# qcraftai/gedepth

Measured on AMD Instinct MI355X. Metric: training img/s (whole node), KITTI-shaped 352x1120 synthetic batches, higher is better.
Workload: dtype bf16; 1 GPU; depthformer_swint_v: DepthFormer-SwinT + GEDepth-Vanilla, 352x1120, 8 img/GPU, full train step; global_batch=8, parallelism=dp1, allreduce_dtype=fp32, layout=nhwc, window_attention=bf16 mfma, params=53516992, hip_graph=off

## Files before the change

### gedepth_amd/csrc/conv1x1_wgrad.hip

```cpp
#include "common.h"
#include <algorithm>

#define C1_ROWS 64
#define C1_MAX_CB 16
#define C1_MAX_IB 3
#define C1_TPW 6
#define C1_DY_PIECES 8
#define C1_X_PIECES 2

__global__ void __launch_bounds__(512, 1) conv1x1_wgrad_k(const bf16_t* __restrict__ x, const bf16_t* __restrict__ dy, float* __restrict__ dw, long M,
                                                          int Ci, int Co, int ci_chunk, int ksplit) {
  __shared__ __attribute__((aligned(16))) bf16_t dy_t[C1_MAX_CB * C1_ROWS * 32];
  __shared__ __attribute__((aligned(16))) bf16_t x_t[C1_MAX_IB * C1_ROWS * 32];
  const int tid = threadIdx.x, lane = tid & 63;
  const int wv = __builtin_amdgcn_readfirstlane(tid >> 6);
  const int ci0 = blockIdx.x * ci_chunk, co0 = blockIdx.y * (C1_MAX_CB * 32);
  const int nib = std::min(ci_chunk, Ci - ci0) >> 5, ncb = std::min(C1_MAX_CB * 32, Co - co0) >> 5;
  const int T = ncb * nib;

  int dy_row[C1_DY_PIECES], dy_col[C1_DY_PIECES], dy_lds[C1_DY_PIECES], x_row[C1_X_PIECES], x_col[C1_X_PIECES], x_lds[C1_X_PIECES];
#pragma unroll
  for (int i = 0; i < C1_DY_PIECES; ++i) {
    const int p = tid + i * 512, ppr = 4 * ncb;
    const int row = p / ppr, part = p - row * ppr;
    dy_row[i] = row < C1_ROWS ? row : -1;
    dy_col[i] = co0 + part * 8;
    dy_lds[i] = ((part >> 2) * C1_ROWS + row) * 32 + (part & 3) * 8;
  }
#pragma unroll
  for (int i = 0; i < C1_X_PIECES; ++i) {
    const int p = tid + i * 512, ppr = 4 * nib;
    const int row = p / ppr, part = p - row * ppr;
    x_row[i] = row < C1_ROWS ? row : -1;
    x_col[i] = ci0 + part * 8;
    x_lds[i] = ((part >> 2) * C1_ROWS + row) * 32 + (part & 3) * 8;
  }
  const int tr_off = ((lane >> 5) * 8 + ((lane & 15) >> 2)) * 32 + ((lane >> 4) & 1) * 16 + (lane & 3) * 4;
  int a_off[C1_TPW], b_off[C1_TPW];
#pragma unroll
  for (int j = 0; j < C1_TPW; ++j) {
    const int t = wv + 8 * j, cb = t / nib, ib = t - cb * nib;
    a_off[j] = cb * C1_ROWS * 32 + tr_off;
    b_off[j] = ib * C1_ROWS * 32 + tr_off;
  }
  ge_f32x16 acc[C1_TPW];
#pragma unroll
  for (int j = 0; j < C1_TPW; ++j) acc[j] = 0.f;

  uint4 pd[C1_DY_PIECES], px[C1_X_PIECES];
  const uint4 zero4 = make_uint4(0, 0, 0, 0);
  const long nstage = (M + C1_ROWS - 1) / C1_ROWS;
#define C1_PREFETCH(S)                                                                                      \
  {                                                                                                         \
    const long r0_ = (long)(S) * C1_ROWS;                                                                   \
    _Pragma("unroll") for (int i = 0; i < C1_DY_PIECES; ++i) {                                             \
      pd[i] = zero4;                                                                                        \
      if (dy_row[i] >= 0 && r0_ + dy_row[i] < M) pd[i] = *(const uint4*)(dy + (r0_ + dy_row[i]) * Co + dy_col[i]);   \
    }                                                                                                       \
    _Pragma("unroll") for (int i = 0; i < C1_X_PIECES; ++i) {                                              \
      px[i] = zero4;                                                                                        \
      if (x_row[i] >= 0 && r0_ + x_row[i] < M) px[i] = *(const uint4*)(x + (r0_ + x_row[i]) * Ci + x_col[i]);        \
    }                                                                                                       \
  }
#define C1_PARK()                                                                                           \
  _Pragma("unroll") for (int i = 0; i < C1_DY_PIECES; ++i) { if (dy_row[i] >= 0) *(uint4*)(dy_t + dy_lds[i]) = pd[i]; }   \
  _Pragma("unroll") for (int i = 0; i < C1_X_PIECES; ++i) { if (x_row[i] >= 0) *(uint4*)(x_t + x_lds[i]) = px[i]; }
#define C1_RD(P) __builtin_shufflevector(__builtin_amdgcn_ds_read_tr16_b64_v4bf16(GE_LDS(ge_bf16x4, (P))), \
                                         __builtin_amdgcn_ds_read_tr16_b64_v4bf16(GE_LDS(ge_bf16x4, (P) + 4 * 32)), 0, 1, 2, 3, 4, 5, 6, 7)
  long s = blockIdx.z;
  if (s < nstage) {
    C1_PREFETCH(s)
    C1_PARK()
  }
  __syncthreads();
  for (; s < nstage; s += ksplit) {
    const bool more = s + ksplit < nstage;
    if (more) { C1_PREFETCH(s + ksplit) }
#pragma unroll
    for (int ks = 0; ks < C1_ROWS / 16; ++ks) {
#pragma unroll
      for (int j = 0; j < C1_TPW; ++j) {
        if (wv + 8 * j < T) {
          const ge_bf16x8 A = C1_RD(dy_t + a_off[j] + ks * 16 * 32);
          const ge_bf16x8 B = C1_RD(x_t + b_off[j] + ks * 16 * 32);
          acc[j] = __builtin_amdgcn_mfma_f32_32x32x16_bf16(A, B, acc[j], 0, 0, 0);
        }
      }
    }
    __syncthreads();
    if (more) { C1_PARK() }
    __syncthreads();
  }
#undef C1_PREFETCH
#undef C1_PARK
#undef C1_RD
#pragma unroll
  for (int j = 0; j < C1_TPW; ++j) {
    const int t = wv + 8 * j;
    if (t < T) {
      const int cb = t / nib, ib = t - cb * nib;
      const int ci = ci0 + ib * 32 + (lane & 31);
#pragma unroll
      for (int r = 0; r < 16; ++r) {
        const int co = co0 + cb * 32 + (r & 3) + 8 * (r >> 2) + 4 * (lane >> 5);
        atomicAdd(dw + (long)co * Ci + ci, acc[j][r]);
      }
    }
  }
}

extern "C" int ge_conv1x1_nhwc_wgrad(const void* x, const void* dy, float* dw, long M, int Cin, int Cout, int dtype, void* stream) {
  if (!x || !dy || !dw || M < 0 || Cin <= 0 || Cout <= 0) return GE_ERR_BAD_ARG;
  if (dtype != GE_BF16 || Cout % 32 || (Cin % 64 && Cin % 96) || (((uintptr_t)x | (uintptr_t)dy) & 15)) return GE_ERR_UNSUPPORTED;
  if (M == 0) return GE_OK;
  const int ci_chunk = (Cin % 96 == 0) ? 96 : 64;
  const int n_ci = Cin / ci_chunk, n_co = (Cout + C1_MAX_CB * 32 - 1) / (C1_MAX_CB * 32);
  if (n_ci > 65535 || n_co > 65535) return GE_ERR_UNSUPPORTED;
  const int cus = ge_cu_count();
  if (!cus) return GE_ERR_BAD_ARG;
  const long nstage = (M + C1_ROWS - 1) / C1_ROWS;
  long ksplit = cus / ((long)n_ci * n_co);
  ksplit = std::max(1L, std::min(ksplit, std::min(nstage, 65535L)));
  const dim3 grid((unsigned)n_ci, (unsigned)n_co, (unsigned)ksplit);
  conv1x1_wgrad_k<<<grid, 512, 0, ge_stream(stream)>>>((const bf16_t*)x, (const bf16_t*)dy, dw, M, Cin, Cout, ci_chunk, (int)ksplit);
  GE_LAUNCH_CHECK();
  return GE_OK;
}
```

### gedepth_amd/hip.py

```python
import ctypes
import os
import re

import torch

_HERE = os.path.dirname(os.path.abspath(__file__))
LIB_PATH = os.environ.get('GE_LIB') or os.path.join(_HERE, 'csrc', 'libgedepth_hip.so')
HEADERS = {'SIGNATURES': 'gedepth_hip.h', 'EVAL_SIGNATURES': 'gedepth_eval.h', 'DDAD_SIGNATURES': 'gedepth_ddad.h',
           'CLOUD_SIGNATURES': 'gedepth_cloud.h', 'GROUND_SIGNATURES': 'gedepth_ground.h'}
EXTRA_HEADERS = {'BATCH_SIGNATURES': 'gedepth_batch.h'}
SCENE_HEADERS = {'SCENE_SIGNATURES': 'gedepth_scene.h'}
STRATA_HEADERS = {'STRATA_SIGNATURES': 'gedepth_strata.h'}
GE_F32, GE_BF16 = 0, 1
GE_COLORIZE_VMIN_DATA, GE_COLORIZE_VMAX_DATA, GE_COLORIZE_EQUAL = 1, 2, 4

_SCALARS = {'int': ctypes.c_int, 'long': ctypes.c_long, 'float': ctypes.c_float, 'double': ctypes.c_double, 'size_t': ctypes.c_size_t,
            'uint64_t': ctypes.c_ulonglong, 'unsigned long long': ctypes.c_ulonglong}
_DECL = re.compile(r'\b(int|size_t)\s+(ge_\w+)\s*\(([^()]*)\)\s*;')


def parse_header(text):
    text = re.sub(r'/\*.*?\*/|//[^\n]*', ' ', text, flags=re.S)
    sigs = {}
    for res, name, params in _DECL.findall(text):
        args = []
        for p in ([] if params.strip() == 'void' else params.split(',')):
            if '*' in p:
                args.append(ctypes.c_void_p)
                continue
            ctype = ' '.join(w for w in p.split()[:-1] if w != 'const')
            if ctype not in _SCALARS:
                raise TypeError(f'{name}: parameter "{" ".join(p.split())}" has a type the ctypes binding does not map')
            args.append(_SCALARS[ctype])
        sigs[name] = (_SCALARS[res], args)
    stray = set(re.findall(r'\b(ge_\w+)\s*\(', text)) - set(sigs)
    if stray:
        raise TypeError(f'cannot parse the declaration of {", ".join(sorted(stray))}')
    return sigs


for _table, _header in {**HEADERS, **EXTRA_HEADERS, **SCENE_HEADERS, **STRATA_HEADERS}.items():
    with open(os.path.join(os.path.dirname(_HERE), 'include', _header)) as _fh:
        globals()[_table] = parse_header(_fh.read())

_lib = None


class HipLibraryError(RuntimeError):
    pass


def lib():
    global _lib
    if _lib is None:
        if not os.path.isfile(LIB_PATH):
            raise HipLibraryError(
                f'{LIB_PATH} is missing: the gfx950 HIP kernels are not built. '
                f'Run gedepth_amd/csrc/build.sh (hipcc --offload-arch=gfx950). There is no CPU/eager fallback.')
        handle = ctypes.CDLL(LIB_PATH)
        for table in (*HEADERS, *EXTRA_HEADERS, *SCENE_HEADERS, *STRATA_HEADERS):
            for name, (res, args) in globals()[table].items():
                fn = getattr(handle, name)
                fn.restype, fn.argtypes = res, args
        _lib = handle
        if os.environ.get('GE_MSDA_MODE'):
            handle.ge_msda_mode(int(os.environ['GE_MSDA_MODE']))
    return _lib


def is_built():
    return os.path.isfile(LIB_PATH)


def check(code, what):
    if code != 0:
        raise RuntimeError(f'{what} failed with code {code} '
                           f'({"bad argument" if code == 10001 else "unsupported" if code == 10002 else "hipError_t"})')


def call(name, *args):
    code = getattr(_lib or lib(), name)(*args)
    if code:
        check(code, name)


def dtype_code(t):
    if t.dtype == torch.float32:
        return GE_F32
    if t.dtype == torch.bfloat16:
        return GE_BF16
    raise TypeError(f'gedepth_amd kernels take float32 or bfloat16 tensors, got {t.dtype}')


def ptr(t, dtype=None, name='tensor'):
    if t is None:
        return None
    if not t.is_cuda:
        raise RuntimeError(f'{name}: gedepth_amd ops run on MI355X only; got a {t.device} tensor '
                           '(the CPU oracle lives in oracle/ and is test infrastructure)')
    if not t.is_contiguous():
        raise RuntimeError(f'{name} must be contiguous')
    if dtype is not None and t.dtype != dtype:
        raise TypeError(f'{name} must be {dtype}, got {t.dtype}')
    return t.data_ptr()


def stream():
    return torch.cuda.current_stream().cuda_stream
```

### gedepth_amd/mmrt/bricks.py

```python
import math
import warnings

import torch
import torch.nn as nn
import torch.nn.functional as F

from .registry import Registry, build_from_cfg

MODELS = Registry('model')
ATTENTION = Registry('attention')
POSITIONAL_ENCODING = Registry('position encoding')
DROPOUT_LAYERS = Registry('drop out layers')


def constant_init(module, val, bias=0):
    if hasattr(module, 'weight') and module.weight is not None:
        nn.init.constant_(module.weight, val)
    if hasattr(module, 'bias') and module.bias is not None:
        nn.init.constant_(module.bias, bias)


def xavier_init(module, gain=1, bias=0, distribution='normal'):
    assert distribution in ['uniform', 'normal']
    if hasattr(module, 'weight') and module.weight is not None:
        if distribution == 'uniform':
            nn.init.xavier_uniform_(module.weight, gain=gain)
        else:
            nn.init.xavier_normal_(module.weight, gain=gain)
    if hasattr(module, 'bias') and module.bias is not None:
        nn.init.constant_(module.bias, bias)


def kaiming_init(module, a=0, mode='fan_out', nonlinearity='relu', bias=0, distribution='normal'):
    assert distribution in ['uniform', 'normal']
    if hasattr(module, 'weight') and module.weight is not None:
        if distribution == 'uniform':
            nn.init.kaiming_uniform_(module.weight, a=a, mode=mode, nonlinearity=nonlinearity)
        else:
            nn.init.kaiming_normal_(module.weight, a=a, mode=mode, nonlinearity=nonlinearity)
    if hasattr(module, 'bias') and module.bias is not None:
        nn.init.constant_(module.bias, bias)


def trunc_normal_init(module, mean=0., std=1., a=-2., b=2., bias=0.):
    if isinstance(module, torch.Tensor):
        nn.init.trunc_normal_(module, mean, std, a, b)
        return
    if hasattr(module, 'weight') and module.weight is not None:
        nn.init.trunc_normal_(module.weight, mean, std, a, b)
    if hasattr(module, 'bias') and module.bias is not None:
        nn.init.constant_(module.bias, bias)


class BaseModule(nn.Module):

    def __init__(self, init_cfg=None):
        super().__init__()
        self._is_init = False
        self.init_cfg = init_cfg

    @property
    def is_init(self):
        return self._is_init

    def init_weights(self):
        if self._is_init:
            warnings.warn(f'init_weights of {self.__class__.__name__} has been called more than once.')
            return
        for m in self.children():
            if hasattr(m, 'init_weights'):
                m.init_weights()
        self._is_init = True


class Sequential(BaseModule, nn.Sequential):

    def __init__(self, *args, init_cfg=None):
        BaseModule.__init__(self, init_cfg)
        nn.Sequential.__init__(self, *args)


class ModuleList(BaseModule, nn.ModuleList):

    def __init__(self, modules=None, init_cfg=None):
        BaseModule.__init__(self, init_cfg)
        nn.ModuleList.__init__(self, modules)


def _split_k(tokens):
    if tokens < 8192:
        return 0
    for s in range(64, 3, -1):
        if tokens % s == 0 and tokens // s >= 1024:
            return s
    return 0


def _linear_fwd(xc, wc, weight, bias, dt):
    from .. import kernels
    from .optim import lowp
    K = xc.shape[-1]
    M = xc.numel() // K
    if (dt == torch.bfloat16 and xc.is_cuda and xc.is_contiguous() and wc.is_contiguous() and kernels.gemm_own(M, K, wc.shape[0])
            and (bias is None or (bias.dtype == torch.float32 and bias.is_contiguous() and bias.data_ptr() % 16 == 0))
            and xc.data_ptr() % 16 == 0 and wc.data_ptr() % 16 == 0):
        return kernels.gemm_nt(xc.reshape(M, K), wc, None if bias is None else bias.detach()).view(*xc.shape[:-1], wc.shape[0])
    return F.linear(xc, wc, None if bias is None else lowp(bias, dt))


def _linear_dx(dy2, wc):
    from .. import kernels
    M, N = dy2.shape
    K = wc.shape[1]
    if dy2.dtype == torch.bfloat16 and dy2.is_contiguous() and dy2.data_ptr() % 16 == 0 and kernels.gemm_own(M, N, K):
        return kernels.gemm_nt(dy2, wc.t().contiguous(), None)
    return dy2 @ wc


def _sum_partials(part, weight, w_dtype):
    if weight is not None and w_dtype == torch.float32:
        from .optim import grad_target
        out = grad_target(weight)
        if out is not None and out.shape == part.shape[1:]:
            return torch.sum(part, 0, dtype=torch.float32, out=out)
    return part.sum(0, dtype=torch.float32).to(w_dtype)


def _plain_dw(dy2, x2, weight, w_dtype):
    if dy2.dtype == torch.bfloat16 and x2.dtype == torch.bfloat16 and w_dtype == torch.float32:
        from .. import kernels
        if 'mm_fp32_out' not in kernels.DISABLED:
            from .optim import grad_target
            out = grad_target(weight) if weight is not None else None
            if out is not None and tuple(out.shape) == (dy2.shape[1], x2.shape[1]):
                return torch.mm(dy2.t(), x2, out_dtype=torch.float32, out=out)
            return torch.mm(dy2.t(), x2, out_dtype=torch.float32)
    return _finished_grad(dy2.t() @ x2, weight, w_dtype)


def _finished_grad(dw, weight, w_dtype):
    from .optim import grad_into_arena
    return grad_into_arena(weight, dw, w_dtype) if weight is not None else dw.to(w_dtype)


class _LinearTokens(torch.autograd.Function):

    @staticmethod
    def forward(ctx, x, weight, bias, splits):
        dt = torch.get_autocast_dtype('cuda') if torch.is_autocast_enabled() else x.dtype
        with torch.autocast('cuda', enabled=False):
            from .optim import lowp
            xc, wc = x.to(dt), lowp(weight, dt)
            y = _linear_fwd(xc, wc, weight, bias, dt)
        ctx.save_for_backward(xc, wc)
        ctx.meta = (splits, x.dtype, weight.dtype, None if bias is None else bias.dtype)
        ctx.weight_ref = weight if isinstance(weight, nn.Parameter) else None
        return y

    @staticmethod
    def backward(ctx, dy):
        xc, wc = ctx.saved_tensors
        splits, x_dtype, w_dtype, b_dtype = ctx.meta
        K = xc.numel() // xc.shape[-1]
        with torch.autocast('cuda', enabled=False):
            dy2 = dy.to(wc.dtype).reshape(K, -1)
            x2 = xc.reshape(K, -1)
            dx = dw = db = None
            if not dy2.is_contiguous():
                dy2 = dy2.contiguous()
            if ctx.needs_input_grad[0]:
                dx = _linear_dx(dy2, wc).reshape(xc.shape).to(x_dtype)
            if ctx.needs_input_grad[1]:
                if splits:
                    M, N = dy2.shape[1], x2.shape[1]
                    part = torch.bmm(dy2.view(splits, K // splits, M).transpose(1, 2), x2.view(splits, K // splits, N))
                    dw = _sum_partials(part, ctx.weight_ref, w_dtype)
                else:
                    dw = _plain_dw(dy2, x2, ctx.weight_ref, w_dtype)
            if b_dtype is not None and ctx.needs_input_grad[2]:
                if dy2.shape[1] % (4 if dy2.dtype == torch.float32 else 8) == 0:
                    from .. import kernels
                    db = kernels.colsum(dy2 if dy2.is_contiguous() else dy2.contiguous()).to(b_dtype)
                else:
                    db = dy2.sum(0, dtype=torch.float32).to(b_dtype)
        return dx, dw, db, None


class _LinearBiasGelu(torch.autograd.Function):

    @staticmethod
    def forward(ctx, x, weight, bias, splits):
        from .. import kernels
        dt = torch.get_autocast_dtype('cuda') if torch.is_autocast_enabled() else x.dtype
        with torch.autocast('cuda', enabled=False):
            from .optim import lowp
            xc, wc = x.to(dt), lowp(weight, dt)
            y0 = _linear_fwd(xc, wc, weight, bias, dt)
            g = kernels.bias_gelu_fwd(y0, None)
        ctx.save_for_backward(xc, wc, y0)
        ctx.meta = (splits, x.dtype, weight.dtype, bias.dtype)
        ctx.weight_ref = weight if isinstance(weight, nn.Parameter) else None
        return g

    @staticmethod
    def backward(ctx, dg):
        from .. import kernels
        xc, wc, y0 = ctx.saved_tensors
        splits, x_dtype, w_dtype, b_dtype = ctx.meta
        K = xc.numel() // xc.shape[-1]
        with torch.autocast('cuda', enabled=False):
            dg2 = dg.to(wc.dtype).reshape(K, -1)
            if not dg2.is_contiguous():
                dg2 = dg2.contiguous()
            dy2, db = kernels.bias_gelu_bwd(dg2, y0.reshape(K, -1), None)
            x2 = xc.reshape(K, -1)
            dx = dw = None
            if ctx.needs_input_grad[0]:
                dx = _linear_dx(dy2, wc).reshape(xc.shape).to(x_dtype)
            if ctx.needs_input_grad[1]:
                if splits:
                    M, N = dy2.shape[1], x2.shape[1]
                    part = torch.bmm(dy2.view(splits, K // splits, M).transpose(1, 2), x2.view(splits, K // splits, N))
                    dw = _sum_partials(part, ctx.weight_ref, w_dtype)
                else:
                    dw = _plain_dw(dy2, x2, ctx.weight_ref, w_dtype)
        return dx, dw, (db.to(b_dtype) if ctx.needs_input_grad[2] else None), None


def linear_bias_gelu(x, weight, bias):
    C = weight.shape[0]
    ok = (x.is_cuda and torch.is_grad_enabled() and weight.requires_grad and bias is not None and x.dim() >= 2 and x.numel() > 0
          and x.dtype in (torch.float32, torch.bfloat16) and C % 8 == 0)
    if ok:
        from .. import kernels
        ok = 'bias_gelu' not in kernels.DISABLED
    if not ok:
        return F.gelu(linear_tokens(x, weight, bias))
    return _LinearBiasGelu.apply(x, weight, bias, _split_k(x.numel() // x.shape[-1]))


def linear_tokens(x, weight, bias=None):
    if not (x.is_cuda and torch.is_grad_enabled() and weight.requires_grad) or x.dtype not in (torch.float32, torch.bfloat16) or x.dim() < 2 or x.numel() == 0:
        return F.linear(x, weight, bias)
    return _LinearTokens.apply(x, weight, bias, _split_k(x.numel() // x.shape[-1]))


class Linear(nn.Linear):

    def forward(self, x):
        return linear_tokens(x, self.weight, self.bias)


class LayerNorm(nn.LayerNorm):
    autocast_out = True

    def _hip_ok(self, x):
        C = x.shape[-1]
        return (x.is_cuda and self.elementwise_affine and len(self.normalized_shape) == 1 and C % 4 == 0 and C <= 3072
                and x.dtype in (torch.float32, torch.bfloat16))

    def _out_dtype(self, x):
        if torch.is_autocast_enabled():
            return torch.get_autocast_dtype('cuda') if self.autocast_out else torch.float32
        return x.dtype

    def forward_with_skip(self, x):
        if self._hip_ok(x) and torch.is_grad_enabled() and x.requires_grad:
            from .. import kernels
            if 'ln_res' not in kernels.DISABLED:
                return kernels.layer_norm_res(x, self.weight, self.bias, self.eps, self._out_dtype(x))
        return self(x), x

    def forward(self, x):
        C = x.shape[-1]
        if self._hip_ok(x):
            from .. import kernels
            return kernels.layer_norm(x, self.weight, self.bias, self.eps, self._out_dtype(x))
        if x.is_cuda:
            from .. import kernels
            kernels.note_fallback('LayerNorm', f'C={C} dtype={x.dtype}')
        return super().forward(x)


_NORM = {
    'BN': ('bn', nn.BatchNorm2d), 'BN1d': ('bn', nn.BatchNorm1d), 'BN2d': ('bn', nn.BatchNorm2d),
    'SyncBN': ('bn', nn.SyncBatchNorm), 'GN': ('gn', nn.GroupNorm), 'LN': ('ln', LayerNorm),
    'IN': ('in', nn.InstanceNorm2d),
}
_ACT = {
    'ReLU': nn.ReLU, 'LeakyReLU': nn.LeakyReLU, 'PReLU': nn.PReLU, 'ReLU6': nn.ReLU6, 'ELU': nn.ELU,
    'Sigmoid': nn.Sigmoid, 'Tanh': nn.Tanh, 'GELU': nn.GELU,
}
_CONV = {'Conv1d': nn.Conv1d, 'Conv2d': nn.Conv2d, 'Conv3d': nn.Conv3d, 'Conv': nn.Conv2d}


def build_norm_layer(cfg, num_features, postfix=''):
    if not isinstance(cfg, dict) or 'type' not in cfg:
        raise KeyError('the cfg dict must contain the key "type"')
    cfg_ = dict(cfg)
    layer_type = cfg_.pop('type')
    if layer_type not in _NORM:
        raise KeyError(f'Unrecognized norm type {layer_type}')
    abbr, norm_layer = _NORM[layer_type]
    name = abbr + str(postfix)
    requires_grad = cfg_.pop('requires_grad', True)
    cfg_.setdefault('eps', 1e-5)
    if layer_type == 'GN':
        assert 'num_groups' in cfg_
        layer = norm_layer(num_channels=num_features, **cfg_)
    else:
        layer = norm_layer(num_features, **cfg_)
    for p in layer.parameters():
        p.requires_grad = requires_grad
    return name, layer


def build_activation_layer(cfg):
    cfg_ = dict(cfg)
    t = cfg_.pop('type')
    if t not in _ACT:
        raise KeyError(f'Unrecognized activation type {t}')
    return _ACT[t](**cfg_)


def build_conv_layer(cfg, *args, **kwargs):
    cfg_ = dict(type='Conv2d') if cfg is None else dict(cfg)
    t = cfg_.pop('type')
    if t not in _CONV:
        raise KeyError(f'Unrecognized conv type {t}')
    return _CONV[t](*args, **kwargs, **cfg_)


class ConvModule(nn.Module):

    def __init__(self, in_channels, out_channels, kernel_size, stride=1, padding=0, dilation=1, groups=1,
                 bias='auto', conv_cfg=None, norm_cfg=None, act_cfg=dict(type='ReLU'), inplace=True,
                 order=('conv', 'norm', 'act')):
        super().__init__()
        assert order == ('conv', 'norm', 'act'), 'only the conv-norm-act order is on the GEDepth path'
        self.conv_cfg, self.norm_cfg, self.act_cfg = conv_cfg, norm_cfg, act_cfg
        self.inplace = inplace
        self.with_norm = norm_cfg is not None
        self.with_activation = act_cfg is not None
        if bias == 'auto':
            bias = not self.with_norm
        self.with_bias = bias
        self.conv = build_conv_layer(conv_cfg, in_channels, out_channels, kernel_size, stride=stride,
                                     padding=padding, dilation=dilation, groups=groups, bias=bias)
        self.in_channels, self.out_channels = in_channels, out_channels
        if self.with_norm:
            self.norm_name, norm = build_norm_layer(norm_cfg, out_channels)
            self.add_module(self.norm_name, norm)
        else:
            self.norm_name = None
        if self.with_activation:
            act_cfg_ = dict(act_cfg)
            if act_cfg_['type'] not in ['Tanh', 'PReLU', 'Sigmoid', 'GELU']:
                act_cfg_.setdefault('inplace', inplace)
            self.activate = build_activation_layer(act_cfg_)
        self.init_weights()

    @property
    def norm(self):
        return getattr(self, self.norm_name) if self.norm_name else None

    def init_weights(self):
        if self.with_activation and self.act_cfg['type'] == 'LeakyReLU':
            nonlinearity, a = 'leaky_relu', self.act_cfg.get('negative_slope', 0.01)
        else:
            nonlinearity, a = 'relu', 0
        kaiming_init(self.conv, a=a, nonlinearity=nonlinearity)
        if self.with_norm:
            constant_init(self.norm, 1, bias=0)
# ... 202 lines not shown
```

### gedepth_amd/mmrt/optim.py

```python
import math

import torch

from .. import hip


class GradArena:

    def __init__(self, params, align=64, adopt=None):
        self.params = [p for p in params if p.requires_grad]
        assert self.params, 'no trainable parameters'
        dev, dt = self.params[0].device, torch.float32
        assert all(p.dtype == dt and p.device == dev for p in self.params), 'fp32 master parameters on one device'
        self.offsets, n = [], 0
        for p in self.params:
            self.offsets.append(n)
            n += (p.numel() + align - 1) // align * align
        self.numel = n
        self.flat_param = torch.zeros(n, device=dev, dtype=dt)
        self.flat_grad = torch.zeros(n, device=dev, dtype=dt)
        self.views = []
        for p, off in zip(self.params, self.offsets):
            view = self._view(self.flat_param, off, p)
            view.copy_(p.data)
            p.data = view
            p.grad = self._view(self.flat_grad, off, p)
            self.views.append(p.grad)
        self.adopt = (dev.type == 'cuda') if adopt is None else bool(adopt)
        self._tag_views()

    def _tag_views(self):
        for p, v in zip(self.params, self.views):
            p._ge_grad_view = v if self.adopt else None

    @staticmethod
    def _view(flat, off, p):
        chunk = flat[off:off + p.numel()]
        if p.dim() == 4 and p.shape[1] > 1 and not p.is_contiguous() and p.is_contiguous(memory_format=torch.channels_last):
            O, I, H, W = p.shape
            return chunk.view(O, H, W, I).permute(0, 3, 1, 2)
        return chunk.view_as(p)

    def zero_grad(self):
        if self.adopt:
            for p in self.params:
                p.grad = None
                p._ge_grad_claimed = False
        else:
            self.flat_grad.zero_()

    def collect(self, indices=None):
        src, dst, empty = [], [], []
        for i in (range(len(self.params)) if indices is None else indices):
            p, v = self.params[i], self.views[i]
            g = p.grad
            if g is None:
                empty.append(v)
            elif g is not v and g.data_ptr() != v.data_ptr():
                src.append(g.detach())
                dst.append(v)
            p.grad = v
            p._ge_grad_claimed = False
        with torch.no_grad():
            if empty:
                torch._foreach_zero_(empty)
            if src:
                torch._foreach_copy_(dst, src)

    def enable_shadow(self):
        if getattr(self, 'flat_shadow', None) is None:
            self.flat_shadow = torch.zeros(self.numel, device=self.flat_param.device, dtype=torch.bfloat16)
            for p, off in zip(self.params, self.offsets):
                p._ge_lp = self._view(self.flat_shadow, off, p)
                p._ge_lp_version = -1
        return self.flat_shadow

    def refresh_shadow(self, copy=True):
        if getattr(self, 'flat_shadow', None) is None:
            return
        if copy:
            self.flat_shadow.copy_(self.flat_param)
        for p in self.params:
            p._ge_lp_version = p._version

    def reattach(self):
        self.collect()

    def slices(self):
        return [(off, p.numel()) for p, off in zip(self.params, self.offsets)]

    def on_permute(self, callback):
        self._permute_callbacks = getattr(self, '_permute_callbacks', []) + [callback]

    @torch.no_grad()
    def permute(self, order):
        n = len(self.params)
        assert sorted(order) == list(range(n)), 'permute() needs a permutation of the parameter indices'
        if list(order) == list(range(n)):
            return
        align_sizes = [(self.offsets[i + 1] if i + 1 < n else self.numel) - self.offsets[i] for i in range(n)]
        old_off = list(self.offsets)
        new_off, pos = [0] * n, 0
        for j, i in enumerate(order):
            new_off[j] = pos
            pos += align_sizes[i]
        assert pos == self.numel
        src = torch.empty(self.numel, dtype=torch.int64)
        for j, i in enumerate(order):
            src[new_off[j]:new_off[j] + align_sizes[i]] = torch.arange(old_off[i], old_off[i] + align_sizes[i])
        src = src.to(self.flat_param.device)

        def remap(buf):
            assert buf.numel() == self.numel
            return buf.index_select(0, src)
        has_grad = [p.grad is not None for p in self.params]
        self.collect()
        self.flat_param = remap(self.flat_param)
        self.flat_grad = remap(self.flat_grad)
        shadow = getattr(self, 'flat_shadow', None)
        if shadow is not None:
            self.flat_shadow = remap(shadow)
        self.params = [self.params[i] for i in order]
        has_grad = [has_grad[i] for i in order]
        self.offsets = new_off
        self.views = []
        for p, off, hg in zip(self.params, self.offsets, has_grad):
            current = getattr(p, '_ge_lp_version', None) == p._version
            p.data = self._view(self.flat_param, off, p)
            view = self._view(self.flat_grad, off, p)
            self.views.append(view)
            p.grad = view if (hg or not self.adopt) else None
            if shadow is not None:
                p._ge_lp = self._view(self.flat_shadow, off, p)
                p._ge_lp_version = p._version if current else -1
        self._tag_views()
        for cb in getattr(self, '_permute_callbacks', []):
            cb(remap)


def _claim(p):
    if getattr(p, '_ge_grad_claimed', False):
        return False
    p._ge_grad_claimed = True
    return True


def grad_target(p, dtype=torch.float32):
    v = getattr(p, '_ge_grad_view', None)
    if v is None or p.grad is not None or v.dtype != dtype or not v.is_contiguous() or not _claim(p):
        return None
    return v.detach()


def grad_target_ohwi(p):
    v = getattr(p, '_ge_grad_view', None)
    if v is None or p.grad is not None or v.dtype != torch.float32 or v.dim() != 4:
        return None
    t = v.detach().permute(0, 2, 3, 1)
    if not t.is_contiguous() or not _claim(p):
        return None
    return t


def grad_into_arena(p, src, dtype=None):
    v = getattr(p, '_ge_grad_view', None) if p is not None else None
    if v is None or p.grad is not None or v.shape != src.shape or not _claim(p):
        return src.to(dtype or (p.dtype if p is not None else src.dtype))
    t = v.detach()
    t.copy_(src)
    return t


def lowp(p, dtype):
    s = getattr(p, '_ge_lp', None)
    if s is not None and s.dtype == dtype and p._ge_lp_version == p._version:
        return s
    return p.to(dtype)


class FusedAdamW(torch.optim.Optimizer):

    def __init__(self, params, lr=1e-3, betas=(0.9, 0.999), eps=1e-8, weight_decay=1e-2, max_grad_norm=0.0, bf16_shadow=True):
        defaults = dict(lr=lr, betas=betas, eps=eps, weight_decay=weight_decay)
        super().__init__(params, defaults)
        wds = sorted({g['weight_decay'] for g in self.param_groups})
        nz = [w for w in wds if w != 0]
        if len(nz) > 1:
            raise NotImplementedError('FusedAdamW supports one non-zero weight decay (decay_mult in {0, 1})')
        self.base_wd = nz[0] if nz else 0.0
        self._check_shared_lr()
        all_params = [p for g in self.param_groups for p in g['params'] if p.requires_grad]
        self.arena = GradArena(all_params)
        dev = self.arena.flat_param.device
        if dev.type != 'cuda':
            raise RuntimeError('FusedAdamW runs on MI355X only (no CPU fallback)')
        self.exp_avg = torch.zeros_like(self.arena.flat_param)
        self.exp_avg_sq = torch.zeros_like(self.arena.flat_param)
        self.wd_mask = torch.zeros(self.arena.numel, device=dev, dtype=torch.uint8)
        decay = {id(p) for g in self.param_groups if g['weight_decay'] != 0 for p in g['params']}
        for p, (off, n) in zip(self.arena.params, self.arena.slices()):
            if id(p) in decay:
                self.wd_mask[off:off + n] = 1
        self.max_grad_norm = float(max_grad_norm)
        self.step_count = 0
        self.hyper = torch.zeros(10, device=dev, dtype=torch.float32)
        self._ring = [(torch.zeros(10, dtype=torch.float32).pin_memory(), torch.cuda.Event()) for _ in range(8)]
        self.gnorm_sq = torch.zeros(1, device=dev, dtype=torch.float64)
        if bf16_shadow:
            self.arena.enable_shadow()
            self.arena.refresh_shadow(copy=True)
        self.arena.on_permute(self._arena_permuted)

    def _check_shared_lr(self):
        lrs = {g['lr'] for g in self.param_groups}
        if len(lrs) > 1:
            raise NotImplementedError(f'FusedAdamW applies one learning rate to the whole arena; the parameter groups have {sorted(lrs)} '
                                      '(lr_mult is not supported)')

    def _arena_permuted(self, remap):
        self.exp_avg, self.exp_avg_sq, self.wd_mask = remap(self.exp_avg), remap(self.exp_avg_sq), remap(self.wd_mask)

    def sync_grads_from_params(self):
        self.arena.reattach()

    def zero_grad(self, set_to_none=False):
        self.arena.zero_grad()

    @property
    def last_grad_norm(self):
        return self.gnorm_sq.sqrt()

    @torch.no_grad()
    def prepare(self):
        g0 = self.param_groups[0]
        self._check_shared_lr()
        self.step_count += 1
        b1, b2 = g0['betas']
        t = self.step_count
        host, ev = self._ring[t % len(self._ring)]
        ev.synchronize()
        host.copy_(torch.tensor([g0['lr'], b1, b2, g0['eps'], self.base_wd, 1 - b1 ** t, 1 - b2 ** t,
                                 self.max_grad_norm, 1 - b1, 1 - b2], dtype=torch.float32))
        self.hyper.copy_(host, non_blocking=True)
        ev.record()

    @torch.no_grad()
    def launch(self):
        a = self.arena
        a.collect()
        self.gnorm_sq.zero_()
        hip.call('ge_sumsq', hip.ptr(a.flat_grad), a.numel, hip.ptr(self.gnorm_sq), hip.stream())
        shadow = getattr(a, 'flat_shadow', None)
        if shadow is None:
            hip.call('ge_adamw_step', hip.ptr(a.flat_param), hip.ptr(a.flat_grad), hip.ptr(self.exp_avg), hip.ptr(self.exp_avg_sq),
                     hip.ptr(self.wd_mask), hip.ptr(self.hyper), hip.ptr(self.gnorm_sq), a.numel, hip.stream())
        else:
            hip.call('ge_adamw_step_shadow', hip.ptr(a.flat_param), hip.ptr(a.flat_grad), hip.ptr(self.exp_avg), hip.ptr(self.exp_avg_sq),
                     hip.ptr(self.wd_mask), hip.ptr(self.hyper), hip.ptr(self.gnorm_sq), a.numel, hip.ptr(shadow), hip.stream())
            a.refresh_shadow(copy=False)

    @torch.no_grad()
    def step(self, closure=None):
        assert closure is None
        self.prepare()
        self.launch()

    def state_dict(self):
        index = {id(p): i for i, p in enumerate(p for g in self.param_groups for p in g['params'])}
        state = {}
        for p, (off, n) in zip(self.arena.params, self.arena.slices()):
            state[index[id(p)]] = dict(step=torch.tensor(float(self.step_count)),
                                       exp_avg=GradArena._view(self.exp_avg, off, p).clone(),
                                       exp_avg_sq=GradArena._view(self.exp_avg_sq, off, p).clone())
        groups = []
        for g in self.param_groups:
            d = {k: v for k, v in g.items() if k != 'params'}
            d['params'] = [index[id(p)] for p in g['params']]
            groups.append(d)
        return dict(state=state, param_groups=groups)

    def load_state_dict(self, state_dict):
        if 'state' not in state_dict:
            for k in ('exp_avg', 'exp_avg_sq'):
                if tuple(state_dict[k].shape) != (self.arena.numel,):
                    raise ValueError(f'optimizer {k}: arena of {tuple(state_dict[k].shape)} elements, this model needs {self.arena.numel}')
            self.step_count = int(state_dict['step'])
            for k, buf in (('exp_avg', self.exp_avg), ('exp_avg_sq', self.exp_avg_sq)):
                src = state_dict[k].to(buf.device, torch.float32)
                buf.zero_()
                for p, (off, n) in zip(self.arena.params, self.arena.slices()):
                    GradArena._view(buf, off, p).copy_(src[off:off + n].view(p.shape))
            for g, s in zip(self.param_groups, state_dict['param_groups']):
                g.update({k: v for k, v in s.items() if k != 'params'})
            return
        saved_groups = state_dict['param_groups']
        if len(saved_groups) != len(self.param_groups):
            raise ValueError(f'optimizer state has {len(saved_groups)} parameter groups, this optimizer {len(self.param_groups)}')
        own_ids, id_of = [], {}
        for g, sg in zip(self.param_groups, saved_groups):
            if len(g['params']) != len(sg['params']):
                raise ValueError('optimizer state: a parameter group has a different number of parameters')
            for p, pid in zip(g['params'], sg['params']):
                id_of[id(p)] = pid
        st = state_dict['state']
# ... 88 lines not shown
```

Baseline: 172.1 img/s.

## Route Swin linear weight grads through custom MFMA wgrad kernel with fused bias sum

Generalizes the 1x1-conv weight-gradient kernel into a templated kernel with selectable output-channel chunk width, an XCD-aware flattened grid and a cost-model planner for chunking and k-split. It also fuses the bias gradient via an MFMA against a ones vector. The kernel is exposed as ge_linear_wgrad and used in the linear backward for a table of (Cin,Cout,M) shapes matching the Swin layers, writing directly into the gradient arena. The optimizer pre-zeroes these gradient views in one foreach call, which replaces the separate bmm/colsum and copy passes. Costs are atomic fp32 accumulation, shape-range gating, and extra bookkeeping for zeroing state.

```diff
diff --git a/gedepth_amd/csrc/conv1x1_wgrad.hip b/gedepth_amd/csrc/conv1x1_wgrad.hip
--- a/gedepth_amd/csrc/conv1x1_wgrad.hip
+++ b/gedepth_amd/csrc/conv1x1_wgrad.hip
@@ -1,22 +1,29 @@
 #include "common.h"
+#include "../../include/gedepth_train.h"
 #include <algorithm>
-
-#define C1_ROWS 64
-#define C1_MAX_CB 16
+#include <cstdio>
+#include <cstdlib>
+
 #define C1_MAX_IB 3
-#define C1_TPW 6
 #define C1_DY_PIECES 8
-#define C1_X_PIECES 2
-
-__global__ void __launch_bounds__(512, 1) conv1x1_wgrad_k(const bf16_t* __restrict__ x, const bf16_t* __restrict__ dy, float* __restrict__ dw, long M,
-                                                          int Ci, int Co, int ci_chunk, int ksplit) {
+#define C1_ROWS_OF(CBW) (128 / (CBW))
+
+template <int C1_CBW>
+__global__ void __launch_bounds__(512, 1) conv1x1_wgrad_k(const bf16_t* __restrict__ x, const bf16_t* __restrict__ dy, float* __restrict__ dw,
+                                                          float* __restrict__ db, long M, int Ci, int Co, int ci_chunk, int co_chunk, int ksplit,
+                                                          int n_ci, int n_co) {
+  constexpr int C1_ROWS = C1_ROWS_OF(C1_CBW);
+  constexpr int C1_MAX_CB = 8 * C1_CBW;
+  constexpr int C1_X_PIECES = C1_CBW == 1 ? 3 : 2;
   __shared__ __attribute__((aligned(16))) bf16_t dy_t[C1_MAX_CB * C1_ROWS * 32];
   __shared__ __attribute__((aligned(16))) bf16_t x_t[C1_MAX_IB * C1_ROWS * 32];
   const int tid = threadIdx.x, lane = tid & 63;
   const int wv = __builtin_amdgcn_readfirstlane(tid >> 6);
-  const int ci0 = blockIdx.x * ci_chunk, co0 = blockIdx.y * (C1_MAX_CB * 32);
-  const int nib = std::min(ci_chunk, Ci - ci0) >> 5, ncb = std::min(C1_MAX_CB * 32, Co - co0) >> 5;
-  const int T = ncb * nib;
+  const int unit = (int)(blockIdx.x >> 3) / n_ci * 8 + (int)(blockIdx.x & 7), bx = (int)(blockIdx.x >> 3) % n_ci;
+  if (unit >= ksplit * n_co) return;
+  const int kz = unit / n_co, by = unit - kz * n_co;
+  const int ci0 = bx * ci_chunk, co0 = by * co_chunk;
+  const int nib = std::min(ci_chunk, Ci - ci0) >> 5, ncb = std::min(co_chunk, Co - co0) >> 5;
 
   int dy_row[C1_DY_PIECES], dy_col[C1_DY_PIECES], dy_lds[C1_DY_PIECES], x_row[C1_X_PIECES], x_col[C1_X_PIECES], x_lds[C1_X_PIECES];
 #pragma unroll
@@ -36,16 +43,22 @@
     x_lds[i] = ((part >> 2) * C1_ROWS + row) * 32 + (part & 3) * 8;
   }
   const int tr_off = ((lane >> 5) * 8 + ((lane & 15) >> 2)) * 32 + ((lane >> 4) & 1) * 16 + (lane & 3) * 4;
-  int a_off[C1_TPW], b_off[C1_TPW];
-#pragma unroll
-  for (int j = 0; j < C1_TPW; ++j) {
-    const int t = wv + 8 * j, cb = t / nib, ib = t - cb * nib;
-    a_off[j] = cb * C1_ROWS * 32 + tr_off;
-    b_off[j] = ib * C1_ROWS * 32 + tr_off;
-  }
-  ge_f32x16 acc[C1_TPW];
-#pragma unroll
-  for (int j = 0; j < C1_TPW; ++j) acc[j] = 0.f;
+  bool own[C1_CBW], sums[C1_CBW];
+#pragma unroll
+  for (int j = 0; j < C1_CBW; ++j) {
+    own[j] = wv + 8 * j < ncb;
+    sums[j] = db != nullptr && own[j] && ((co0 >> 5) + wv + 8 * j) % n_ci == bx;
+  }
+  ge_f32x16 acc[C1_CBW][C1_MAX_IB], accb[C1_CBW];
+#pragma unroll
+  for (int j = 0; j < C1_CBW; ++j) {
+    accb[j] = 0.f;
+#pragma unroll
+    for (int ib = 0; ib < C1_MAX_IB; ++ib) acc[j][ib] = 0.f;
+  }
+  ge_bf16x8 ones;
+#pragma unroll
+  for (int i = 0; i < 8; ++i) ones[i] = (__bf16)1.f;
 
   uint4 pd[C1_DY_PIECES], px[C1_X_PIECES];
   const uint4 zero4 = make_uint4(0, 0, 0, 0);
@@ -67,7 +80,7 @@
   _Pragma("unroll") for (int i = 0; i < C1_X_PIECES; ++i) { if (x_row[i] >= 0) *(uint4*)(x_t + x_lds[i]) = px[i]; }
 #define C1_RD(P) __builtin_shufflevector(__builtin_amdgcn_ds_read_tr16_b64_v4bf16(GE_LDS(ge_bf16x4, (P))), \
                                          __builtin_amdgcn_ds_read_tr16_b64_v4bf16(GE_LDS(ge_bf16x4, (P) + 4 * 32)), 0, 1, 2, 3, 4, 5, 6, 7)
-  long s = blockIdx.z;
+  long s = kz;
   if (s < nstage) {
     C1_PREFETCH(s)
     C1_PARK()
@@ -76,14 +89,21 @@
   for (; s < nstage; s += ksplit) {
     const bool more = s + ksplit < nstage;
     if (more) { C1_PREFETCH(s + ksplit) }
-#pragma unroll
-    for (int ks = 0; ks < C1_ROWS / 16; ++ks) {
-#pragma unroll
-      for (int j = 0; j < C1_TPW; ++j) {
-        if (wv + 8 * j < T) {
-          const ge_bf16x8 A = C1_RD(dy_t + a_off[j] + ks * 16 * 32);
-          const ge_bf16x8 B = C1_RD(x_t + b_off[j] + ks * 16 * 32);
-          acc[j] = __builtin_amdgcn_mfma_f32_32x32x16_bf16(A, B, acc[j], 0, 0, 0);
+    if (own[0]) {
+#pragma unroll
+      for (int ks = 0; ks < C1_ROWS / 16; ++ks) {
+        ge_bf16x8 B[C1_MAX_IB];
+#pragma unroll
+        for (int ib = 0; ib < C1_MAX_IB; ++ib) B[ib] = ib < nib ? C1_RD(x_t + (ib * C1_ROWS + ks * 16) * 32 + tr_off) : ones;
+#pragma unroll
+        for (int j = 0; j < C1_CBW; ++j) {
+          if (own[j]) {
+            const ge_bf16x8 A = C1_RD(dy_t + ((wv + 8 * j) * C1_ROWS + ks * 16) * 32 + tr_off);
+#pragma unroll
+            for (int ib = 0; ib < C1_MAX_IB; ++ib)
+              if (ib < nib) acc[j][ib] = __builtin_amdgcn_mfma_f32_32x32x16_bf16(A, B[ib], acc[j][ib], 0, 0, 0);
+            if (sums[j]) accb[j] = __builtin_amdgcn_mfma_f32_32x32x16_bf16(A, ones, accb[j], 0, 0, 0);
+          }
         }
       }
     }
@@ -95,34 +115,104 @@
 #undef C1_PARK
 #undef C1_RD
 #pragma unroll
-  for (int j = 0; j < C1_TPW; ++j) {
-    const int t = wv + 8 * j;
-    if (t < T) {
-      const int cb = t / nib, ib = t - cb * nib;
-      const int ci = ci0 + ib * 32 + (lane & 31);
-#pragma unroll
-      for (int r = 0; r < 16; ++r) {
-        const int co = co0 + cb * 32 + (r & 3) + 8 * (r >> 2) + 4 * (lane >> 5);
-        atomicAdd(dw + (long)co * Ci + ci, acc[j][r]);
-      }
-    }
-  }
-}
-
-extern "C" int ge_conv1x1_nhwc_wgrad(const void* x, const void* dy, float* dw, long M, int Cin, int Cout, int dtype, void* stream) {
+  for (int j = 0; j < C1_CBW; ++j) {
+    if (own[j]) {
+      const int cob = co0 + (wv + 8 * j) * 32 + 4 * (lane >> 5);
+#pragma unroll
+      for (int ib = 0; ib < C1_MAX_IB; ++ib) {
+        if (ib < nib) {
+          const int ci = ci0 + ib * 32 + (lane & 31);
+#pragma unroll
+          for (int r = 0; r < 16; ++r) atomicAdd(dw + (long)(cob + (r & 3) + 8 * (r >> 2)) * Ci + ci, acc[j][ib][r]);
+        }
+      }
+      if (sums[j] && (lane & 31) == 0) {
+#pragma unroll
+        for (int r = 0; r < 16; ++r) atomicAdd(db + cob + (r & 3) + 8 * (r >> 2), accb[j][r]);
+      }
+    }
+  }
+}
+
+struct C1Plan { int ci_chunk, co_chunk, ksplit, n_ci, n_co; };
+static C1Plan c1_plan(long M, int Cin, int Cout, int cus) {
+  C1Plan best = {0, 0, 0, 0, 0};
+  double best_t = 0.0;
+  const int ci_chunk = (Cin % 96 == 0) ? 96 : 64, n_ci = Cin / ci_chunk;
+  if (const char* ev = getenv("GE_LINEAR_WGRAD_PLAN")) {
+    int co = 0, ks = 0;
+    if (sscanf(ev, "%d,%d", &co, &ks) == 2 && (co == 128 || co == 256 || co == 512) && ks >= 1) {
+      const long nstage = (M + C1_ROWS_OF(co / 512 + 1) - 1) / C1_ROWS_OF(co / 512 + 1);
+      ks = (int)std::min((long)ks, std::min(nstage, 65535L));
+      return {ci_chunk, co, ks, n_ci, (Cout + co - 1) / co};
+    }
+  }
+  for (int co_chunk = 128; co_chunk <= 512; co_chunk *= 2) {
+    const int rows = C1_ROWS_OF(co_chunk / 512 + 1);
+    const long nstage = (M + rows - 1) / rows;
+    const int n_co = (Cout + co_chunk - 1) / co_chunk;
+    const long blocks = (long)n_ci * n_co;
+    const double t_l2 = (double)M * 2.0 * ((double)Cout * n_ci + (double)Cin * n_co) / 15e12;
+    const double t_stage = 0.9e-6 + (double)rows * (std::min(co_chunk, Cout) + ci_chunk) * 2.0 / 54e9;
+    const long ks_max = std::max(1L, std::min(std::min(nstage, 65535L), 2L * cus / blocks));
+    for (long ks = 1; ks <= ks_max; ++ks) {
+      const long per_xcd = (ks * n_co + 7) / 8 * n_ci, cus_xcd = std::max(1, cus / 8);
+      const long rounds = (per_xcd + cus_xcd - 1) / cus_xcd, per_wg = (nstage + ks - 1) / ks;
+      const double t_wg = (double)rounds * per_wg * t_stage;
+      const double t_hbm = (double)M * 2.0 * (Cout + Cin) / std::min(4.5e12, (double)std::min(blocks * ks, (long)cus) * 24e9) +
+                           (double)M * 2.0 * Cin * (n_co - 1) / 8.6e12;
+      const double t = std::max(std::max(t_hbm, t_l2), t_wg) + (double)ks * Cout * Cin / 64.0 / 5.1e9;
+      if (!best.ksplit || t < best_t) {
+        best_t = t;
+        best = {ci_chunk, co_chunk, (int)ks, n_ci, n_co};
+      }
+    }
+    if (Cout <= co_chunk) break;
+  }
+  return best;
+}
+
+static int c1_check(const void* x, const void* dy, const float* dw, const float* db, long M, int Cin, int Cout, int dtype) {
   if (!x || !dy || !dw || M < 0 || Cin <= 0 || Cout <= 0) return GE_ERR_BAD_ARG;
-  if (dtype != GE_BF16 || Cout % 32 || (Cin % 64 && Cin % 96) || (((uintptr_t)x | (uintptr_t)dy) & 15)) return GE_ERR_UNSUPPORTED;
+  if (dtype != GE_BF16 || Cout % 32 || (Cin % 64 && Cin % 96) || (((uintptr_t)x | (uintptr_t)dy) & 15) || (((uintptr_t)dw | (uintptr_t)db) & 3))
+    return GE_ERR_UNSUPPORTED;
+  return GE_OK;
+}
+
+static int c1_launch(const void* x, const void* dy, float* dw, float* db, long M, int Cin, int Cout, void* stream) {
   if (M == 0) return GE_OK;
-  const int ci_chunk = (Cin % 96 == 0) ? 96 : 64;
-  const int n_ci = Cin / ci_chunk, n_co = (Cout + C1_MAX_CB * 32 - 1) / (C1_MAX_CB * 32);
-  if (n_ci > 65535 || n_co > 65535) return GE_ERR_UNSUPPORTED;
   const int cus = ge_cu_count();
   if (!cus) return GE_ERR_BAD_ARG;
-  const long nstage = (M + C1_ROWS - 1) / C1_ROWS;
-  long ksplit = cus / ((long)n_ci * n_co);
-  ksplit = std::max(1L, std::min(ksplit, std::min(nstage, 65535L)));
-  const dim3 grid((unsigned)n_ci, (unsigned)n_co, (unsigned)ksplit);
-  conv1x1_wgrad_k<<<grid, 512, 0, ge_stream(stream)>>>((const bf16_t*)x, (const bf16_t*)dy, dw, M, Cin, Cout, ci_chunk, (int)ksplit);
+  const C1Plan p = c1_plan(M, Cin, Cout, cus);
+  const long units = ((long)p.ksplit * p.n_co + 7) / 8 * 8;
+  if (units * p.n_ci > 0x7fffffffL) return GE_ERR_UNSUPPORTED;
+  const dim3 grid((unsigned)(units * p.n_ci));
+  if (p.co_chunk > 256)
+    conv1x1_wgrad_k<2><<<grid, 512, 0, ge_stream(stream)>>>((const bf16_t*)x, (const bf16_t*)dy, dw, db, M, Cin, Cout, p.ci_chunk, p.co_chunk, p.ksplit,
+                                                            p.n_ci, p.n_co);
+  else
+    conv1x1_wgrad_k<1><<<grid, 512, 0, ge_stream(stream)>>>((const bf16_t*)x, (const bf16_t*)dy, dw, db, M, Cin, Cout, p.ci_chunk, p.co_chunk, p.ksplit,
+                                                            p.n_ci, p.n_co);
   GE_LAUNCH_CHECK();
   return GE_OK;
 }
+
+extern "C" int ge_conv1x1_nhwc_wgrad(const void* x, const void* dy, float* dw, long M, int Cin, int Cout, int dtype, void* stream) {
+  const int e = c1_check(x, dy, dw, nullptr, M, Cin, Cout, dtype);
+  return e ? e : c1_launch(x, dy, dw, nullptr, M, Cin, Cout, stream);
+}
+
+extern "C" int ge_linear_wgrad(const void* x, const void* dy, float* dw, float* db, long M, int Cin, int Cout, int dtype, void* stream) {
+  const int e = c1_check(x, dy, dw, db, M, Cin, Cout, dtype);
+  return e ? e : c1_launch(x, dy, dw, db, M, Cin, Cout, stream);
+}
+
+extern "C" int ge_linear_wgrad_plan(long M, int Cin, int Cout, int* plan) {
+  if (!plan || M <= 0 || Cin <= 0 || Cout <= 0) return GE_ERR_BAD_ARG;
+  if (Cout % 32 || (Cin % 64 && Cin % 96)) return GE_ERR_UNSUPPORTED;
+  const int cus = ge_cu_count();
+  if (!cus) return GE_ERR_BAD_ARG;
+  const C1Plan p = c1_plan(M, Cin, Cout, cus);
+  plan[0] = p.ci_chunk; plan[1] = p.co_chunk; plan[2] = p.ksplit;
+  return GE_OK;
+}
diff --git a/gedepth_amd/hip.py b/gedepth_amd/hip.py
--- a/gedepth_amd/hip.py
+++ b/gedepth_amd/hip.py
@@ -11,6 +11,7 @@
 EXTRA_HEADERS = {'BATCH_SIGNATURES': 'gedepth_batch.h'}
 SCENE_HEADERS = {'SCENE_SIGNATURES': 'gedepth_scene.h'}
 STRATA_HEADERS = {'STRATA_SIGNATURES': 'gedepth_strata.h'}
+TRAIN_HEADERS = {'TRAIN_SIGNATURES': 'gedepth_train.h'}
 GE_F32, GE_BF16 = 0, 1
 GE_COLORIZE_VMIN_DATA, GE_COLORIZE_VMAX_DATA, GE_COLORIZE_EQUAL = 1, 2, 4
 
@@ -39,7 +40,7 @@
     return sigs
 
 
-for _table, _header in {**HEADERS, **EXTRA_HEADERS, **SCENE_HEADERS, **STRATA_HEADERS}.items():
+for _table, _header in {**HEADERS, **EXTRA_HEADERS, **SCENE_HEADERS, **STRATA_HEADERS, **TRAIN_HEADERS}.items():
     with open(os.path.join(os.path.dirname(_HERE), 'include', _header)) as _fh:
         globals()[_table] = parse_header(_fh.read())
 
@@ -58,7 +59,7 @@
                 f'{LIB_PATH} is missing: the gfx950 HIP kernels are not built. '
                 f'Run gedepth_amd/csrc/build.sh (hipcc --offload-arch=gfx950). There is no CPU/eager fallback.')
         handle = ctypes.CDLL(LIB_PATH)
-        for table in (*HEADERS, *EXTRA_HEADERS, *SCENE_HEADERS, *STRATA_HEADERS):
+        for table in (*HEADERS, *EXTRA_HEADERS, *SCENE_HEADERS, *STRATA_HEADERS, *TRAIN_HEADERS):
             for name, (res, args) in globals()[table].items():
                 fn = getattr(handle, name)
                 fn.restype, fn.argtypes = res, args
diff --git a/gedepth_amd/mmrt/bricks.py b/gedepth_amd/mmrt/bricks.py
--- a/gedepth_amd/mmrt/bricks.py
+++ b/gedepth_amd/mmrt/bricks.py
@@ -143,6 +143,39 @@
     return grad_into_arena(weight, dw, w_dtype) if weight is not None else dw.to(w_dtype)
 
 
+def _own_wgrad_ok(dy2, x2, w_dtype):
+    if not (dy2.is_cuda and dy2.dtype == torch.bfloat16 and x2.dtype == torch.bfloat16 and w_dtype == torch.float32):
+        return False
+    from .. import train_kernels
+    return (train_kernels.linear_wgrad_own(x2.shape[0], x2.shape[1], dy2.shape[1]) and x2.is_contiguous() and dy2.is_contiguous()
+            and x2.data_ptr() % 16 == 0 and dy2.data_ptr() % 16 == 0)
+
+
+def _own_wgrad(dy2, x2, weight, bias, want_db):
+    from .. import train_kernels
+    from .optim import grad_target, take_prezeroed
+    Cout, Cin = dy2.shape[1], x2.shape[1]
+    tw = grad_target(weight) if weight is not None else None
+    if tw is not None and tuple(tw.shape) != (Cout, Cin):
+        tw = None
+    tb = None
+    if tw is None:
+        buf = torch.zeros(Cout * Cin + (Cout if want_db else 0), device=dy2.device, dtype=torch.float32)
+        tw = buf[:Cout * Cin].view(Cout, Cin)
+        tb = buf[Cout * Cin:] if want_db else None
+    else:
+        zeroed = take_prezeroed(weight)
+        if want_db and bias is not None and getattr(weight, '_ge_grad_follower', None) is bias:
+            tb = grad_target(bias)
+        if tb is not None:
+            if not (take_prezeroed(bias) and zeroed):
+                torch.as_strided(tw, ((tb.data_ptr() - tw.data_ptr()) // 4 + Cout,), (1,)).zero_()
+        elif not zeroed:
+            tw.zero_()
+    train_kernels.linear_wgrad(x2, dy2, tw, tb)
+    return tw, tb
+
+
 class _LinearTokens(torch.autograd.Function):
 
     @staticmethod
@@ -155,6 +188,7 @@
         ctx.save_for_backward(xc, wc)
         ctx.meta = (splits, x.dtype, weight.dtype, None if bias is None else bias.dtype)
         ctx.weight_ref = weight if isinstance(weight, nn.Parameter) else None
+        ctx.bias_ref = bias if isinstance(bias, nn.Parameter) else None
         return y
 
     @staticmethod
@@ -170,14 +204,19 @@
                 dy2 = dy2.contiguous()
             if ctx.needs_input_grad[0]:
                 dx = _linear_dx(dy2, wc).reshape(xc.shape).to(x_dtype)
+            want_db = b_dtype is not None and ctx.needs_input_grad[2]
             if ctx.needs_input_grad[1]:
-                if splits:
+                if _own_wgrad_ok(dy2, x2, w_dtype):
+                    dw, db = _own_wgrad(dy2, x2, ctx.weight_ref, ctx.bias_ref, want_db and b_dtype == torch.float32)
+                    if db is not None:
+                        want_db = False
+                elif splits:
                     M, N = dy2.shape[1], x2.shape[1]
                     part = torch.bmm(dy2.view(splits, K // splits, M).transpose(1, 2), x2.view(splits, K // splits, N))
                     dw = _sum_partials(part, ctx.weight_ref, w_dtype)
                 else:
                     dw = _plain_dw(dy2, x2, ctx.weight_ref, w_dtype)
-            if b_dtype is not None and ctx.needs_input_grad[2]:
+            if want_db:
                 if dy2.shape[1] % (4 if dy2.dtype == torch.float32 else 8) == 0:
                     from .. import kernels
                     db = kernels.colsum(dy2 if dy2.is_contiguous() else dy2.contiguous()).to(b_dtype)
@@ -218,7 +257,9 @@
             if ctx.needs_input_grad[0]:
                 dx = _linear_dx(dy2, wc).reshape(xc.shape).to(x_dtype)
             if ctx.needs_input_grad[1]:
-                if splits:
+                if _own_wgrad_ok(dy2, x2, w_dtype):
+                    dw, _ = _own_wgrad(dy2, x2, ctx.weight_ref, None, False)
+                elif splits:
                     M, N = dy2.shape[1], x2.shape[1]
                     part = torch.bmm(dy2.view(splits, K // splits, M).transpose(1, 2), x2.view(splits, K // splits, N))
                     dw = _sum_partials(part, ctx.weight_ref, w_dtype)
diff --git a/gedepth_amd/mmrt/optim.py b/gedepth_amd/mmrt/optim.py
--- a/gedepth_amd/mmrt/optim.py
+++ b/gedepth_amd/mmrt/optim.py
@@ -30,8 +30,9 @@
         self._tag_views()
 
     def _tag_views(self):
-        for p, v in zip(self.params, self.views):
+        for i, (p, v) in enumerate(zip(self.params, self.views)):
             p._ge_grad_view = v if self.adopt else None
+            p._ge_grad_follower = self.params[i + 1] if self.adopt and i + 1 < len(self.params) else None
 
     @staticmethod
     def _view(flat, off, p):
@@ -43,9 +44,16 @@
 
     def zero_grad(self):
         if self.adopt:
+            pre = []
             for p in self.params:
                 p.grad = None
                 p._ge_grad_claimed = False
+                if getattr(p, '_ge_grad_prezero', False):
+                    pre.append(p._ge_grad_view)
+                    p._ge_grad_zeroed = True
+            if pre:
+                with torch.no_grad():
+                    torch._foreach_zero_(pre)
         else:
             self.flat_grad.zero_()
 
@@ -61,6 +69,7 @@
                 dst.append(v)
             p.grad = v
             p._ge_grad_claimed = False
+            p._ge_grad_zeroed = False
         with torch.no_grad():
             if empty:
                 torch._foreach_zero_(empty)
@@ -150,6 +159,13 @@
     if v is None or p.grad is not None or v.dtype != dtype or not v.is_contiguous() or not _claim(p):
         return None
     return v.detach()
+
+
+def take_prezeroed(p):
+    zeroed = getattr(p, '_ge_grad_zeroed', False)
+    p._ge_grad_zeroed = False
+    p._ge_grad_prezero = True
+    return zeroed
 
 
 def grad_target_ohwi(p):
diff --git a/gedepth_amd/train_kernels.py b/gedepth_amd/train_kernels.py
--- /dev/null
+++ b/gedepth_amd/train_kernels.py
@@ -0,0 +1,46 @@
+import ctypes
+import os
+
+import torch
+
+from . import hip, kernels
+
+LINEAR_WGRAD_OWN = {
+    (192, 192): (40000, 60000),
+    (384, 1152): (10000, 16000),
+    (384, 384): (10000, 16000),
+    (1536, 384): (10000, 16000),
+    (768, 384): (10000, 16000),
+    (768, 768): (2500, 4000),
+}
+_ALL = os.environ.get('GE_LINEAR_WGRAD', '') == 'all'
+
+
+def linear_wgrad_supported(M, Cin, Cout):
+    return M > 0 and Cout % 32 == 0 and (Cin % 64 == 0 or Cin % 96 == 0)
+
+
+def linear_wgrad_own(M, Cin, Cout):
+    if 'linear_wgrad' in kernels.DISABLED or not linear_wgrad_supported(M, Cin, Cout):
+        return False
+    if _ALL:
+        return True
+    r = LINEAR_WGRAD_OWN.get((Cin, Cout))
+    return r is not None and r[0] <= M <= r[1]
+
+
+def linear_wgrad_plan(M, Cin, Cout):
+    plan = (ctypes.c_int * 3)()
+    hip.check(hip.lib().ge_linear_wgrad_plan(M, Cin, Cout, ctypes.cast(plan, ctypes.c_void_p)), 'ge_linear_wgrad_plan')
+    return tuple(plan)
+
+
+def linear_wgrad(x2, dy2, dw, db=None):
+    M, Cin = x2.shape
+    Cout = dy2.shape[1]
+    assert dy2.shape[0] == M and tuple(dw.shape) == (Cout, Cin) and (db is None or tuple(db.shape) == (Cout,))
+    nbytes = (x2.numel() + dy2.numel()) * 2 + 2 * 4 * (dw.numel() + (0 if db is None else db.numel()))
+    kernels._launch(f'linear_wgrad[{M}x{Cin}->{Cout}{"" if db is None else " +db"}]', nbytes, 'ge_linear_wgrad',
+                    hip.ptr(x2, torch.bfloat16, 'x'), hip.ptr(dy2, torch.bfloat16, 'dy'), hip.ptr(dw, torch.float32, 'dw'),
+                    hip.ptr(db, torch.float32, 'db'), M, Cin, Cout, hip.GE_BF16, hip.stream(), flops=2 * M * Cin * Cout)
+    return dw, db
diff --git a/include/gedepth_train.h b/include/gedepth_train.h
--- /dev/null
+++ b/include/gedepth_train.h
@@ -0,0 +1,15 @@
+#ifndef GEDEPTH_TRAIN_H
+#define GEDEPTH_TRAIN_H
+
+#ifdef __cplusplus
+extern "C" {
+#endif
+
+int ge_linear_wgrad(const void* x, const void* dy, float* dw, float* db, long M, int Cin, int Cout, int dtype, void* stream);
+
+int ge_linear_wgrad_plan(long M, int Cin, int Cout, int* plan);
+
+#ifdef __cplusplus
+}
+#endif
+#endif
```

Result: no change. 173.0 img/s (median of 6 runs) (+0.5%).
